# AssemblyAI-Community/MinImagen

Hardware: NVIDIA H100
Metric: denoising steps/sec (SR256 U-Net, batch 32 per GPU per step) (higher is better)
Workload: dtype f16 tensor-core operands, f32 accumulate / residual stream

## Files before the change

include/minimagen_b200.h:

```cpp
#ifndef MINIMAGEN_B200_H_
#define MINIMAGEN_B200_H_

#include <stdint.h>

#ifdef __cplusplus
extern "C" {
#endif

#define MI_ABI_VERSION 2

int mi_abi_version(void);
const char* mi_last_error(void);
int mi_device_ok(void);
int mi_set_launch_mode(int programmatic_dependent_launch);

int mi_pack_conv_weight_f16(const float* w_oihw, int c_out, int c_in, int kh, int kw, float scale, void* out_f16,
                            void* stream);

int mi_pack_conv_weight_dgrad_f16(const float* w_oihw, int c_out, int c_in, int kh, int kw, void* out_f16, void* stream);

int mi_conv2d_igemm_supported(int H, int W, int c_in, int c_out);
int mi_conv2d_igemm_f16(const void* act_f16, int B, int H, int W, int lda, int c_off, int c_in, const void* act2_f16,
                        int lda2, int c_off2, int c_in1, const void* w_f16, int c_out, int kh, int kw, int mode,
                        const float* bias, const float* residual, float* out_f32, void* out_f16, double* out_stats,
                        long long out_sb, long long out_sh, long long out_sw, long long out_sc, int n_valid,
                        int block_n, int* err_flag, void* workspace, long long workspace_bytes, void* stream);
int mi_conv3x3_res1x1_supported(int H, int W, int c_in, int c_out, int x_cin);
int mi_conv3x3_res1x1_f16(const void* act_f16, int B, int H, int W, int lda, int c_in, const void* act2_f16, int lda2,
                          int c_in1, const void* x_f16, int ldx, int x_cin, const void* x2_f16, int ldx2, int x_cin1,
                          const void* w_f16, int c_out, const float* bias, const float* residual, float* out_f32,
                          void* out_f16, double* out_stats, int* err_flag, void* stream);
long long mi_conv2d_igemm_workspace_bytes(void);

int mi_conv3x3_gn_supported(int H, int W, int c0, int c1, int c_out, int groups);
int mi_conv3x3_gn_silu_f16(const float* src0, int c0, const float* src1, int c1, float scale1, int B, int H, int W,
                           int groups, const double* stats0, const double* stats1, const float* gamma,
                           const float* beta, const float* scale_shift, int scale_shift_ld, float eps,
                           const void* w_f16, int c_out, const float* bias, const float* residual, float* out_f32,
                           void* out_f16, double* out_stats, int* err_flag, void* stream);

int mi_conv2d_direct_f32(const float* in, int B, int Hin, int Win, int c_in, int ldi, const float* w_oihw, int c_out,
// ... 104 lines not shown
```

minimagen_b200/_native.py:

```python
import ctypes
import os
from ctypes import c_char_p, c_float, c_int, c_longlong, c_void_p

import torch

_HERE = os.path.dirname(os.path.abspath(__file__))
LIB_PATH = os.path.join(_HERE, "lib", "libminimagen_b200.so")

_P, _I, _L, _F = c_void_p, c_int, c_longlong, c_float

SIGNATURES = {
    "mi_abi_version": [],
    "mi_last_error": [],
    "mi_device_ok": [],
    "mi_set_launch_mode": [_I],
    "mi_pack_conv_weight_f16": [_P, _I, _I, _I, _I, _F, _P, _P],
    "mi_pack_conv_weight_dgrad_f16": [_P, _I, _I, _I, _I, _P, _P],
    "mi_conv2d_igemm_supported": [_I, _I, _I, _I],
    "mi_conv2d_igemm_f16": [_P, _I, _I, _I, _I, _I, _I, _P, _I, _I, _I, _P, _I, _I, _I, _I, _P, _P, _P, _P, _P, _L, _L, _L, _L,
                            _I, _I, _P, _P, _L, _P],
    "mi_conv3x3_res1x1_supported": [_I, _I, _I, _I, _I],
    "mi_conv3x3_res1x1_f16": [_P, _I, _I, _I, _I, _I, _P, _I, _I, _P, _I, _I, _P, _I, _I, _P, _I, _P, _P, _P, _P, _P, _P, _P],
    "mi_conv2d_igemm_workspace_bytes": [],
    "mi_conv3x3_gn_supported": [_I, _I, _I, _I, _I, _I],
    "mi_conv3x3_gn_silu_f16": [_P, _I, _P, _I, _F, _I, _I, _I, _I, _P, _P, _P, _P, _P, _I, _F, _P, _I, _P, _P, _P, _P, _P, _P,
                               _P],
    "mi_conv2d_direct_f32": [_P, _I, _I, _I, _I, _I, _P, _I, _I, _I, _I, _I, _P, _P, _P, _I, _I, _L, _L, _L, _L, _P],
    "mi_gn_stats": [_P, _I, _P, _I, _F, _I, _I, _I, _I, _P, _P],
    "mi_gn_apply_silu": [_P, _I, _P, _I, _F, _I, _I, _I, _I, _P, _I, _P, _I, _P, _P, _P, _I, _F, _P, _I, _P],
    "mi_cast_act": [_P, _I, _P, _I, _F, _I, _I, _I, _I, _I, _P, _I, _P],
    "mi_ln_rows": [_P, _L, _I, _P, _P, _F, _I, _P, _P, _P, _P],
    "mi_linear_f32": [_P, _I, _I, _P, _P, _I, _I, _I, _P, _P, _P, _F, _P],
    "mi_sinusoidal_posemb": [_P, _I, _I, _P, _P],
    "mi_text_tokens": [_P, _I, _I, _I, _P, _P, _P, _I, _P, _I, _I, _P, _P],
    "mi_place_rows": [_P, _I, _I, _I, _P, _I, _I, _P],
# ... 109 lines not shown
```

minimagen_b200/csrc/capi.cu:

```cuda
#include "../../include/minimagen_b200.h"

#include <cuda_runtime.h>
#include <stdio.h>
#include <stdlib.h>
#include <string.h>
#include <string>

#include "conv_tc.cuh"
#include "kernels.cuh"

namespace {

thread_local char g_err[256] = "ok";

int fail(int code, const char* what) {
    snprintf(g_err, sizeof(g_err), "%s (code %d)", what, code);
    return code;
}
int check(int rc, const char* fn) {
    if (rc == 0) return 0;
    if (rc == -1) return fail(rc, (std::string(fn) + ": unsupported shape / alignment").c_str());
    if (rc == -2) {
        cudaError_t e = cudaGetLastError();
        return fail(rc, (std::string(fn) + ": kernel launch failed: " + cudaGetErrorString(e)).c_str());
// ... 27 lines not shown

int mi_pack_conv_weight_dgrad_f16(const float* w, int c_out, int c_in, int kh, int kw, void* out, void* stream) {
    return check(mi::pack_conv_weight_dgrad(w, c_out, c_in, kh, kw, (__half*)out, S(stream)), "mi_pack_conv_weight_dgrad_f16");
}
int mi_pack_conv_weight_f16(const float* w, int c_out, int c_in, int kh, int kw, float scale, void* out, void* stream) {
    return check(mi::pack_conv_weight(w, c_out, c_in, kh, kw, scale, (__half*)out, S(stream)), "mi_pack_conv_weight_f16");
}

int mi_conv2d_igemm_supported(int H, int W, int c_in, int c_out) { return mi::conv_tc_supported(H, W, c_in, c_out) ? 1 : 0; }

static int igemm_common(const void* act, int B, int H, int W, int lda, int c_off, int c_in, const void* act2, int lda2,
                        int c_off2, int c_in1, const void* w, int c_out, int kh, int kw, int mode, const float* bias,
                        const float* residual, float* out_f32, void* out_f16, double* out_stats, long long out_sb,
                        long long out_sh, long long out_sw, long long out_sc, int n_valid, int block_n, int* err_flag,
                        void* workspace, long long workspace_bytes, const void* x_act, int ldx, int x_off, int x_cin,
                        const void* x_act2, int ldx2, int x_off2, int x_cin1, void* stream) {
    mi::ConvTcProblem p{};
    p.x_act = x_act; p.x_lda = ldx; p.x_chan_off = x_off; p.Cx = x_cin;
    p.x_act2 = x_act2; p.x_lda2 = ldx2; p.x_chan_off2 = x_off2; p.Cx1 = x_cin1;
    if (x_act && !(mode == 0 && kh == 3 && kw == 3)) return fail(-9, "mi_conv3x3_res1x1_f16: the folded 1x1 operand needs a 3x3 stride-1 conv");
    (void)workspace; (void)workspace_bytes;
    p.act = act; p.B = B; p.H = H; p.W = W; p.lda = lda; p.a_channels = lda; p.a_chan_off = c_off; p.Cin = c_in;
    p.wpacked = w; p.Cout = c_out;
    p.act2 = act2; p.lda2 = lda2; p.a_chan_off2 = c_off2; p.Cin1 = c_in1; p.stats = out_stats;
    if (out_stats && (out_sc > 1 || (c_out % 32) != 0)) return fail(-8, "mi_conv2d_igemm_f16: out_stats needs channel-contiguous output and c_out % 32 == 0");
    if (out_stats && ((long long)H * W) % 32 != 0)
        return fail(-8, "mi_conv2d_igemm_f16: out_stats needs H*W % 32 == 0 (a warp's output rows must belong to one image)");
    p.out_f32 = out_f32; p.out_f16 = (__half*)out_f16; p.bias = bias; p.residual = residual;
    p.out_sb = out_sb; p.out_sh = out_sh; p.out_sw = out_sw; p.out_sc = out_sc; p.n_valid = n_valid;
    p.block_n_hint = block_n; p.err_flag = err_flag;
    if (mode == 0) {
        if (!(kh & 1) || !(kw & 1) || kh * kw > mi::kConvMaxTaps) return fail(-4, "mi_conv2d_igemm_f16: mode 0 needs odd kh,kw with kh*kw <= 16");
// ... 36 lines not shown
    if (out_sc <= 1 && ((out_sw % 4) || (out_sh % 4) || (out_sb % 4)))
        return fail(-8, "mi_conv2d_igemm_f16: channel-contiguous output strides must be multiples of 4 elements");
    if (out_sc > 1 && residual) return fail(-8, "mi_conv2d_igemm_f16: residual needs channel-contiguous output");
    const int rc = mi::conv_tc_launch(p, S(stream));
    if (rc != 0) return fail(rc, mi::conv_tc_strerror(rc));
    return 0;
}

int mi_conv2d_igemm_f16(const void* act, int B, int H, int W, int lda, int c_off, int c_in, const void* act2, int lda2,
                        int c_off2, int c_in1, const void* w, int c_out, int kh, int kw, int mode, const float* bias,
                        const float* residual, float* out_f32, void* out_f16, double* out_stats, long long out_sb,
                        long long out_sh, long long out_sw, long long out_sc, int n_valid, int block_n, int* err_flag,
                        void* workspace, long long workspace_bytes, void* stream) {
    return igemm_common(act, B, H, W, lda, c_off, c_in, act2, lda2, c_off2, c_in1, w, c_out, kh, kw, mode, bias, residual,
                        out_f32, out_f16, out_stats, out_sb, out_sh, out_sw, out_sc, n_valid, block_n, err_flag, workspace,
                        workspace_bytes, nullptr, 0, 0, 0, nullptr, 0, 0, 0, stream);
}

int mi_conv3x3_res1x1_supported(int H, int W, int c_in, int c_out, int x_cin) {
    const bool t16 = W == 16 && H % 16 == 0, t32 = !t16 && H % 32 == 0 && W % 8 == 0;
    return (t16 || t32) && mi::conv_tc_supported(H, W, c_in, c_out) && x_cin > 0 && x_cin % 64 == 0 && c_out % 128 == 0;
}

int mi_conv3x3_res1x1_f16(const void* act, int B, int H, int W, int lda, int c_in, const void* act2, int lda2, int c_in1,
                          const void* x_act, int ldx, int x_cin, const void* x_act2, int ldx2, int x_cin1, const void* w,
                          int c_out, const float* bias, const float* residual, float* out_f32, void* out_f16,
                          double* out_stats, int* err_flag, void* stream) {
    if (!mi_conv3x3_res1x1_supported(H, W, c_in, c_out, x_cin))
        return fail(-9, "mi_conv3x3_res1x1_f16: unsupported geometry (see mi_conv3x3_res1x1_supported)");
    return igemm_common(act, B, H, W, lda, 0, c_in, act2, lda2, 0, c_in1, w, c_out, 3, 3, 0, bias, residual, out_f32, out_f16,
                        out_stats, (long long)H * W * c_out, (long long)W * c_out, c_out, 1, 0, 0, err_flag, nullptr, 0, x_act,
                        ldx, 0, x_cin, x_act2, ldx2, 0, x_cin1, stream);
}

long long mi_conv2d_igemm_workspace_bytes(void) { return 0; }

int mi_conv3x3_gn_supported(int H, int W, int c0, int c1, int c_out, int groups) {
    return mi::conv_gn_supported(H, W, c0, c1, c_out, groups) ? 1 : 0;
}

int mi_conv3x3_gn_silu_f16(const float* src0, int c0, const float* src1, int c1, float scale1, int B, int H, int W,
                           int groups, const double* stats0, const double* stats1, const float* gamma,
                           const float* beta, const float* scale_shift, int scale_shift_ld, float eps, const void* w,
                           int c_out, const float* bias, const float* residual, float* out_f32, void* out_f16,
                           double* out_stats, int* err_flag, void* stream) {
    mi::ConvGnProblem p{};
    p.src0 = src0; p.C0 = c0; p.src1 = src1; p.C1 = c1; p.scale1 = scale1; p.B = B; p.H = H; p.W = W; p.groups = groups;
// ... 214 lines not shown
```

minimagen_b200/csrc/conv_tc.cu:

```cuda
#include "conv_tc.cuh"

#include <cuda_runtime.h>
#include <mutex>
#include <stdio.h>

#include "kernels.cuh"
#include "launch.cuh"
#include "ptx.cuh"
#include "sat_half.cuh"
#include "wgmma.cuh"

namespace mi {

namespace {

constexpr int kNumThreads = 384;
constexpr uint32_t kABytes = kConvBlockM * kConvBlockK * 2;
constexpr uint32_t kRingBudget = 192 * 1024;
constexpr uint32_t kAuxBytes = 512;
constexpr uint32_t kSmemMax = 227 * 1024;
constexpr int kProducerRegs = 40;
constexpr int kConsumerRegs = 232;
static_assert(128 * kProducerRegs + 256 * kConsumerRegs <= 65536, "register file overcommitted");
constexpr int kTurnBar = 2;
constexpr int kStatBar = 4;
constexpr uint32_t stat_scratch_bytes(int block_n) { return 2 * 4 * (block_n / 16 > 0 ? block_n / 16 : 1) * 2 * 8; }

template <int BLOCK_N>
struct Cfg {
    static constexpr uint32_t kBBytes = BLOCK_N * kConvBlockK * 2;
    static constexpr uint32_t kStageBytes = kABytes + kBBytes;
    static constexpr int kStages = (kRingBudget / kStageBytes) > 8 ? 8 : (kRingBudget / kStageBytes);
    static constexpr uint32_t kSmemBytes = kStages * kStageBytes + 1024  + kAuxBytes;
};

__device__ __forceinline__ float silu(float v) { return __fdividef(v, 1.0f + __expf(-v)); }

template <int BLOCK_N, bool GN>
__global__ void __launch_bounds__(kNumThreads, 1)
conv_wg_kernel(const __grid_constant__ CUtensorMap tmA, const __grid_constant__ CUtensorMap tmA2,
               const __grid_constant__ CUtensorMap tmB, const __grid_constant__ CUtensorMap tmX,
               const __grid_constant__ CUtensorMap tmX2, const __grid_constant__ ConvTcArgs args,
               const __grid_constant__ GnPrologueArgs gn) {
    using C = Cfg<BLOCK_N>;
    constexpr int STAGES = C::kStages;
    static_assert(2 * STAGES * 8 <= 256, "barrier block overlaps the GroupNorm scratch");
    constexpr bool PP = !GN && BLOCK_N <= 128;
    constexpr int HALVES = PP ? 2 : 1;

    extern __shared__ uint8_t smem_raw[];
    uint8_t* smem = reinterpret_cast<uint8_t*>((reinterpret_cast<uintptr_t>(smem_raw) + 1023) & ~uintptr_t(1023));
    uint64_t* bars = reinterpret_cast<uint64_t*>(smem + STAGES * C::kStageBytes);
    uint64_t* full_bar = bars;
    uint64_t* empty_bar = bars + STAGES;

    const int warp = threadIdx.x >> 5;
    const int lane = threadIdx.x & 31;
    const int wg = threadIdx.x >> 7;
    int* err = args.err_flag;

    if (threadIdx.x == 0) {
        ptx::prefetch_tensormap(&tmB);
        if (!GN) {
// ... 22 lines not shown
            if (warp == 0) {
                int stage = 0;
                uint32_t phase = 0;
                for (int tile = blockIdx.x; tile < total_tiles; tile += gridDim.x) {
                    const int nt = tile % args.tiles_n;
                    const int mt = tile / args.tiles_n;
                    const int w0 = (mt % args.tiles_w) * BW;
                    const int h0 = ((mt / args.tiles_w) % args.tiles_h) * BH;
                    const int b0 = (mt / (args.tiles_w * args.tiles_h)) * BB;
                    const int n0 = nt * BLOCK_N;
                    for (int kb = 0; kb < num_kb; ++kb) {
                        ptx::mbar_wait(&empty_bar[stage], phase ^ 1, err, 100 + stage);
                        if (ptx::elect_one()) {
                            uint8_t* sa = smem + stage * C::kStageBytes;
                            uint8_t* sb = sa + kABytes;
                            ptx::mbar_arrive_expect_tx(&full_bar[stage], C::kStageBytes);
                            if (kb < num_tap_kb) {
                                const int t = kb / args.chunks_per_tap, j = kb - t * args.chunks_per_tap;
                                const int cw = w0 * args.in_stride + args.dw[t], ch = h0 * args.in_stride + args.dh[t];
                                if (j < args.a_split)
                                    ptx::tma_load_5d(&tmA, &full_bar[stage], sa, args.a_chan_off + j * kConvBlockK, cw, ch,
                                                     args.ph[t], b0);
                                else
                                    ptx::tma_load_5d(&tmA2, &full_bar[stage], sa,
                                                     args.a_chan_off2 + (j - args.a_split) * kConvBlockK, cw, ch, args.ph[t], b0);
                            } else {
                                const int jx = kb - num_tap_kb;
                                if (jx < args.x_split)
                                    ptx::tma_load_5d(&tmX, &full_bar[stage], sa, args.x_chan_off + jx * kConvBlockK, w0, h0, 0, b0);
                                else
                                    ptx::tma_load_5d(&tmX2, &full_bar[stage], sa,
                                                     args.x_chan_off2 + (jx - args.x_split) * kConvBlockK, w0, h0, 0, b0);
                            }
                            ptx::tma_load_2d(&tmB, &full_bar[stage], sb, kb * kConvBlockK, n0);
                        }
                        if (++stage == STAGES) { stage = 0; phase ^= 1; }
                    }
                }
                pdl_trigger();
            }
        } else {
            float* s_mean = reinterpret_cast<float*>(reinterpret_cast<uint8_t*>(bars) + 256);
            float* s_rstd = s_mean + 32;
            float* sA = reinterpret_cast<float*>(reinterpret_cast<uint8_t*>(bars) + kAuxBytes);
            const int tt = threadIdx.x;
            const int lq = tt & 7;
            const int prow = tt >> 3;
            const int C0 = gn.C0, C1 = gn.C1, Ctot = C0 + C1, Cg = Ctot / gn.groups;
            const int H = args.H, W = args.W;
// ... 120 lines not shown
        if (PP) skip(cw * num_kb);
        int bw_r[2 * HALVES], bh_r[2 * HALVES], bb_r[2 * HALVES], bb_warp[HALVES];
#pragma unroll
        for (int h = 0; h < HALVES; ++h) {
            const int m_warp = (PP ? h : cw) * 64 + wq * 16;
            bb_warp[h] = m_warp >> (args.bw_log2 + args.bh_log2);
#pragma unroll
            for (int r = 0; r < 2; ++r) {
                const int m = m_warp + (lane >> 2) + 8 * r;
                bw_r[2 * h + r] = m & (BW - 1);
                bh_r[2 * h + r] = (m >> args.bw_log2) & (BH - 1);
                bb_r[2 * h + r] = m >> (args.bw_log2 + args.bh_log2);
            }
        }
        constexpr int NQ = BLOCK_N / 16 > 0 ? BLOCK_N / 16 : 1;
        const bool tile_stats = PP && args.stats != nullptr && BB == 1;
        double* st_red = reinterpret_cast<double*>(reinterpret_cast<uint8_t*>(bars) + kAuxBytes);
        const bool vec = args.out_sc == 1 && ((reinterpret_cast<uintptr_t>(args.out_f32) & 7) == 0) &&
                         ((reinterpret_cast<uintptr_t>(args.residual) & 7) == 0) &&
                         ((reinterpret_cast<uintptr_t>(args.out_f16) & 3) == 0);

        for (int tile = blockIdx.x + (PP ? cw : 0) * gridDim.x; tile < total_tiles; tile += (PP ? 2 : 1) * gridDim.x) {
            const int nt = tile % args.tiles_n;
            const int mt = tile / args.tiles_n;
            const int n0 = nt * BLOCK_N;
            if (PP && tile != (int)blockIdx.x) ptx::bar_sync(kTurnBar + cw, 256);
            int prev = -1;
            for (int kb = 0; kb < num_kb; ++kb) {
                ptx::mbar_wait(&full_bar[stage], phase, err, 300 + stage);
                const uint32_t sa = ptx::smem_u32(smem + stage * C::kStageBytes);
                const uint64_t db = ptx::make_sw128_desc(sa + kABytes);
                ptx::wg_fence();
#pragma unroll
                for (int k = 0; k < kConvBlockK / 16; ++k)
#pragma unroll
                    for (int h = 0; h < HALVES; ++h) {
                        const uint64_t da = ptx::make_sw128_desc(sa + (PP ? h : cw) * (64 * 128));
                        ptx::Wgmma<BLOCK_N, 0>::run(acc[h], da + 2 * k, db + 2 * k, (kb | k) != 0);
                    }
                ptx::wg_commit();
                ptx::wg_wait<1>();
                if (prev >= 0 && (threadIdx.x & 127) == 0) ptx::mbar_arrive(&empty_bar[prev]);
                prev = stage;
                if (++stage == STAGES) { stage = 0; phase ^= 1; }
            }
            if (PP && tile + (int)gridDim.x < total_tiles) ptx::bar_arrive(kTurnBar + (cw ^ 1), 256);
            if (PP) skip(num_kb);
            ptx::wg_wait<0>();
#pragma unroll
            for (int h = 0; h < HALVES; ++h) ptx::wg_fence_regs(acc[h]);
            if (prev >= 0 && (threadIdx.x & 127) == 0) ptx::mbar_arrive(&empty_bar[prev]);

            const int tw0 = (mt % args.tiles_w) * BW;
            const int th0 = ((mt / args.tiles_w) % args.tiles_h) * BH;
            const int tb0 = (mt / (args.tiles_w * args.tiles_h)) * BB;
// ... 2 lines not shown
            for (int hf = 0; hf < HALVES; ++hf) {
                bool valid[2];
                long long pix[2];
#pragma unroll
                for (int r = 0; r < 2; ++r) {
                    const int w = tw0 + bw_r[2 * hf + r], h = th0 + bh_r[2 * hf + r], b = tb0 + bb_r[2 * hf + r];
                    valid[r] = (b < args.B) && (h < args.H) && (w < args.W);
                    pix[r] = (long long)b * args.out_sb + (long long)h * args.out_sh + (long long)w * args.out_sw;
                }
                const float* a = acc[hf];
                float st_s[BLOCK_N / 16 > 0 ? BLOCK_N / 16 : 1], st_q[BLOCK_N / 16 > 0 ? BLOCK_N / 16 : 1];
#pragma unroll
                for (int q = 0; q < BLOCK_N / 16; ++q) { st_s[q] = 0.f; st_q[q] = 0.f; }
#pragma unroll
                for (int j = 0; j < BLOCK_N / 8; ++j) {
                    const int n = n0 + 8 * j + cq;
                    if (fast) {
                        float2 bv = make_float2(0.f, 0.f);
                        if (args.bias) bv = __ldg(reinterpret_cast<const float2*>(args.bias + n));
#pragma unroll
                        for (int r = 0; r < 2; ++r) {
                            if (!valid[r]) continue;
                            const long long o = pix[r] + n;
                            float2 f = make_float2(a[4 * j + 2 * r] + bv.x, a[4 * j + 2 * r + 1] + bv.y);
                            if (args.residual) {
                                const float2 rv = *reinterpret_cast<const float2*>(args.residual + o);
                                f.x += rv.x; f.y += rv.y;
                            }
                            st_s[j >> 1] += f.x + f.y;
                            st_q[j >> 1] += f.x * f.x + f.y * f.y;
                            if (args.out_f32) *reinterpret_cast<float2*>(args.out_f32 + o) = f;
// ... 19 lines not shown
                if (args.stats) {
                    const int b_img = tb0 + bb_warp[hf];
                    const bool any = __any_sync(0xffffffffu, valid[0] || valid[1]);
#pragma unroll
                    for (int q = 0; q < BLOCK_N / 16; ++q) {
#pragma unroll
                        for (int o = 1; o <= 16; o <<= 1) {
                            st_s[q] += __shfl_xor_sync(0xffffffffu, st_s[q], o);
                            st_q[q] += __shfl_xor_sync(0xffffffffu, st_q[q], o);
                        }
                        if (lane == 0 && tile_stats) {
                            double* r = st_red + ((cw * 4 + wq) * NQ + q) * 2;
                            r[0] = (hf == 0 ? 0.0 : r[0]) + (double)st_s[q];
                            r[1] = (hf == 0 ? 0.0 : r[1]) + (double)st_q[q];
                        } else if (lane == 0 && any) {
                            double* dst = args.stats + ((long long)b_img * args.stats_blocks + (n0 >> 4) + q) * 2;
                            atomicAdd(dst, (double)st_s[q]);
                            atomicAdd(dst + 1, (double)st_q[q]);
                        }
                    }
                }
            }
            if (tile_stats) {
                ptx::bar_sync(kStatBar + cw, 128);
                if (wq == 0 && lane < NQ) {
                    const double* r = st_red + (cw * 4 * NQ + lane) * 2;
                    double s = r[0], sq = r[1];
#pragma unroll
                    for (int w = 1; w < 4; ++w) { s += r[w * NQ * 2]; sq += r[w * NQ * 2 + 1]; }
                    double* dst = args.stats + ((long long)tb0 * args.stats_blocks + (n0 >> 4) + lane) * 2;
                    atomicAdd(dst, s);
                    atomicAdd(dst + 1, sq);
                }
                ptx::bar_sync(kStatBar + cw, 128);
            }
        }
    }
}


typedef CUresult (*PFN_encodeTiled)(CUtensorMap*, CUtensorMapDataType, cuuint32_t, void*, const cuuint64_t*,
                                    const cuuint64_t*, const cuuint32_t*, const cuuint32_t*, CUtensorMapInterleave,
                                    CUtensorMapSwizzle, CUtensorMapL2promotion, CUtensorMapFloatOOBfill);

PFN_encodeTiled get_encode() {
// ... 66 lines not shown
    return enc(m, CU_TENSOR_MAP_DATA_TYPE_FLOAT16, 5, const_cast<void*>(ptr), gdim, gstr, box, estr,
               CU_TENSOR_MAP_INTERLEAVE_NONE, CU_TENSOR_MAP_SWIZZLE_128B, CU_TENSOR_MAP_L2_PROMOTION_L2_256B,
               CU_TENSOR_MAP_FLOAT_OOB_FILL_NONE);
}

CUresult encode_weights(PFN_encodeTiled enc, CUtensorMap* m, const void* ptr, cuuint64_t K, int Cout, int block_n) {
    cuuint64_t gdim[2] = {K, (cuuint64_t)Cout};
    cuuint64_t gstr[1] = {K * 2};
    cuuint32_t box[2] = {kConvBlockK, (cuuint32_t)block_n};
    cuuint32_t estr[2] = {1, 1};
    return enc(m, CU_TENSOR_MAP_DATA_TYPE_FLOAT16, 2, const_cast<void*>(ptr), gdim, gstr, box, estr,
               CU_TENSOR_MAP_INTERLEAVE_NONE, CU_TENSOR_MAP_SWIZZLE_128B, CU_TENSOR_MAP_L2_PROMOTION_L2_256B,
               CU_TENSOR_MAP_FLOAT_OOB_FILL_NONE);
}

template <int BLOCK_N, bool GN>
int launch(const CUtensorMap& tmA, const CUtensorMap& tmA2, const CUtensorMap& tmB, const CUtensorMap& tmX,
           const CUtensorMap& tmX2, const ConvTcArgs& args, const GnPrologueArgs& gn, uint32_t extra_smem,
           cudaStream_t stream) {
    using C = Cfg<BLOCK_N>;
    static bool attr_set = false;
    if (!attr_set) {
        if (cudaFuncSetAttribute(conv_wg_kernel<BLOCK_N, GN>, cudaFuncAttributeMaxDynamicSharedMemorySize, kSmemMax) !=
            cudaSuccess)
            return -10;
        attr_set = true;
    }
    const int total_tiles = args.tiles_w * args.tiles_h * args.tiles_b * args.tiles_n;
    const int num_sms = num_sms_of_current_device();
    const int grid = total_tiles < num_sms ? total_tiles : num_sms;
    const uint32_t smem = C::kSmemBytes + (!GN && BLOCK_N <= 128 ? stat_scratch_bytes(BLOCK_N) : 0u) + extra_smem;
    launch_k(conv_wg_kernel<BLOCK_N, GN>, grid, kNumThreads, smem, stream, tmA, tmA2, tmB, tmX, tmX2, args, gn);
    return cudaGetLastError() == cudaSuccess ? 0 : -11;
}

}

PFN_tmaEncodeTiled get_tma_encode() { return get_encode(); }

const char* conv_tc_strerror(int code) {
    switch (code) {
        case 0: return "ok";
        case -1: return "conv_tc: C_in (per tap) must be a positive multiple of 64";
        case -2: return "conv_tc: C_out must be a multiple of 16";
        case -3: return "conv_tc: W must be a power of two >= 8 or a multiple of 128; H*W tiling unsupported";
        case -4: return "conv_tc: too many taps (max 16)";
        case -5: return "conv_tc: cuTensorMapEncodeTiled unavailable";
        case -6: return "conv_tc: tensor map encode failed (activations)";
        case -7: return "conv_tc: tensor map encode failed (weights)";
        case -8: return "conv_tc: pointer/stride alignment (16 B) violated";
        case -9: return "conv_tc: the folded 1x1 operand needs a stride-1 conv over one phase";
        case -10: return "conv_tc: cudaFuncSetAttribute(max dynamic smem) failed";
        case -11: return "conv_tc: kernel launch failed";
        default: return "conv_tc: unknown error";
    }
}

bool conv_tc_supported(int H, int W, int Cin, int Cout) {
    if (Cin <= 0 || Cin % kConvBlockK != 0 || Cout <= 0 || Cout % 16 != 0) return false;
    if (W >= 128) return true;
    if (ilog2_exact(W) < 3) return false;
    const int bh = 128 / W;
    if (H >= bh) return H % bh == 0;
    return ilog2_exact(H) >= 0;
}

int conv_tc_launch(const ConvTcProblem& p, cudaStream_t stream) {
    if (p.Cin <= 0 || p.Cin % kConvBlockK != 0) return -1;
// ... 9 lines not shown
    ConvTcArgs a{};
    a.num_taps = p.num_taps;
    a.chunks_per_tap = p.Cin / kConvBlockK;
    tile_geometry(p.H, p.W, p.B, a);
    a.a_chan_off = p.a_chan_off;
    a.in_stride = p.in_stride == 2 ? 2 : 1;
    a.out_sb = p.out_sb; a.out_sh = p.out_sh; a.out_sw = p.out_sw;
    a.out_sc = p.out_sc > 0 ? p.out_sc : 1;
    a.n_valid = p.n_valid > 0 ? p.n_valid : p.Cout;
    a.out_f32 = p.out_f32; a.out_f16 = p.out_f16; a.bias = p.bias; a.residual = p.residual;
    a.err_flag = p.err_flag;
    a.stats = p.stats; a.stats_blocks = p.Cout / 16;
    for (int t = 0; t < p.num_taps; ++t) { a.dh[t] = p.dh[t]; a.dw[t] = p.dw[t]; a.ph[t] = p.ph[t]; }

    const int tiles_m = a.tiles_w * a.tiles_h * a.tiles_b;
    const int block_n = pick_block_n(p.Cout, tiles_m, p.block_n_hint, num_sms_of_current_device());
    a.tiles_n = p.Cout / block_n;

    CUtensorMap tmA, tmA2, tmB, tmX, tmX2;
    a.a_split = (p.act2 ? p.Cin1 : p.Cin) / kConvBlockK;
    a.a_chan_off2 = p.a_chan_off2;
    if (encode_act(enc, &tmA, p.act, p.a_channels, p.lda, p.W, p.H, p.phases, p.B, a.in_stride, a) != CUDA_SUCCESS) return -6;
    tmA2 = tmA;
    if (p.act2) {
        if (p.Cin1 <= 0 || p.Cin1 % kConvBlockK || p.Cin1 >= p.Cin || (p.lda2 % 8) || (reinterpret_cast<uintptr_t>(p.act2) & 15) ||
            a.in_stride != 1)
            return -8;
        if (encode_act(enc, &tmA2, p.act2, p.lda2, p.lda2, p.W, p.H, p.phases, p.B, 1, a) != CUDA_SUCCESS) return -6;
    }
    tmX = tmA; tmX2 = tmA;
    if (p.x_act) {
// ... 1 lines not shown
        if (p.Cx <= 0 || p.Cx % kConvBlockK || (p.x_lda % 8) || (reinterpret_cast<uintptr_t>(p.x_act) & 15)) return -8;
        if (p.x_act2 && (p.Cx1 <= 0 || p.Cx1 % kConvBlockK || p.Cx1 >= p.Cx || (p.x_lda2 % 8) ||
                         (reinterpret_cast<uintptr_t>(p.x_act2) & 15)))
            return -8;
        a.x_chunks = p.Cx / kConvBlockK;
        a.x_split = (p.x_act2 ? p.Cx1 : p.Cx) / kConvBlockK;
        a.x_chan_off = p.x_chan_off; a.x_chan_off2 = p.x_chan_off2;
        if (encode_act(enc, &tmX, p.x_act, p.x_lda, p.x_lda, p.W, p.H, 1, p.B, 1, a) != CUDA_SUCCESS) return -6;
        tmX2 = tmX;
        if (p.x_act2 && encode_act(enc, &tmX2, p.x_act2, p.x_lda2, p.x_lda2, p.W, p.H, 1, p.B, 1, a) != CUDA_SUCCESS) return -6;
    }
    const cuuint64_t K = (cuuint64_t)p.num_taps * p.Cin + (p.x_act ? (cuuint64_t)p.Cx : 0);
    if (encode_weights(enc, &tmB, p.wpacked, K, p.Cout, block_n) != CUDA_SUCCESS) return -7;

    const GnPrologueArgs gn{};
    switch (block_n) {
        case 256: return launch<256, false>(tmA, tmA2, tmB, tmX, tmX2, a, gn, 0, stream);
        case 128: return launch<128, false>(tmA, tmA2, tmB, tmX, tmX2, a, gn, 0, stream);
        case 64: return launch<64, false>(tmA, tmA2, tmB, tmX, tmX2, a, gn, 0, stream);
        case 32: return launch<32, false>(tmA, tmA2, tmB, tmX, tmX2, a, gn, 0, stream);
        default: return launch<16, false>(tmA, tmA2, tmB, tmX, tmX2, a, gn, 0, stream);
    }
}


bool conv_gn_supported(int H, int W, int C0, int C1, int Cout, int groups) {
    const int C = C0 + C1;
    if (H <= 0 || W <= 0 || H % 32 || W % 8 || C0 <= 0 || C0 % 64 || C1 < 0 || C1 % 64 || Cout <= 0 || Cout % 128) return false;
    if (!conv_tc_supported(H, W, C, Cout) || H * W < kConvBlockM) return false;
    if (groups < 1 || groups > 32 || C % groups) return false;
// ... 41 lines not shown
```

minimagen_b200/csrc/conv_tc.cuh:

```cuda
#pragma once
#include <cuda_fp16.h>
#include <cuda_runtime.h>
#include <stdint.h>

namespace mi {

constexpr int kConvBlockM = 128;
constexpr int kConvBlockK = 64;
constexpr int kConvMaxTaps = 16;

struct ConvTcArgs {
    int num_taps, chunks_per_tap;
    int bw_log2, bh_log2;
    int tiles_w, tiles_h, tiles_b, tiles_n;
    int B, H, W;
    int a_chan_off;
    int in_stride;
    int a_split, a_chan_off2;
    int x_chunks, x_split;
    int x_chan_off, x_chan_off2;
    long long out_sb, out_sh, out_sw;
    long long out_sc;
    int n_valid;
    float* out_f32;
    __half* out_f16;
    const float* bias;
    const float* residual;
    int* err_flag;
    double* stats;
    int stats_blocks;
    int8_t dh[kConvMaxTaps], dw[kConvMaxTaps], ph[kConvMaxTaps];
};

struct ConvTcProblem {
    const void* act;
    int B, H, W;
    int phases;
    int in_stride;
    int lda;
    int a_channels;
    int a_chan_off;
    int Cin;
    const void* act2;
    int lda2, a_chan_off2, Cin1;
    const void* wpacked;
    int Cout;
    const void* x_act; int x_lda, x_chan_off, Cx;
    const void* x_act2; int x_lda2, x_chan_off2, Cx1;
    int num_taps;
    int8_t dh[kConvMaxTaps], dw[kConvMaxTaps], ph[kConvMaxTaps];
    float* out_f32; __half* out_f16; const float* bias; const float* residual;
    long long out_sb, out_sh, out_sw;
    long long out_sc;
    int n_valid;
    int block_n_hint;
    double* stats;
    int* err_flag;
};

struct GnPrologueArgs {
    const float* src0;
    const float* src1;
    int C0, C1, groups;
    float scale1, eps;
    const double* stats0;
    const double* stats1;
    const float* gamma;
    const float* beta;
    const float* scale_shift;
    int ss_ld;
};

// ... 22 lines not shown
```

minimagen_b200/layers.py:

```python
import math
import os

import torch
from torch import nn

from .helpers import default, exists
from .ops import get_ops

F16, F32, F64 = torch.float16, torch.float32, torch.float64


STATS_BLOCK = 16

GN_INPUT_F32 = True

FUSE_GN_CONV = {"0": False, "1": True, "pair": "pair", "all": "all"}.get(os.environ.get("MI_FUSE_GN_CONV", "0"), False)
FUSE_OVER_FOLD = os.environ.get("MI_FUSE_OVER_FOLD", "1") == "1"


def fuse_block_ok(c_out):
    if not FUSE_GN_CONV:
        return False
    if FUSE_GN_CONV == 'all':
        return True
# ... 462 lines not shown

class _UpsampleSeq(nn.Sequential):

    def run(self, x):
        return self[1].run(x, upsample=True, f32=GN_INPUT_F32, f16=True, stats=True)

    def forward(self, x):
        _no_grad_check(x)
        return to_nchw(self.run(to_nhwc(x)).need_f32())


def Upsample(dim, dim_out=None):
    return _UpsampleSeq(nn.Upsample(scale_factor=2, mode='nearest'), Conv2d(dim, default(dim_out, dim), 3, padding=1))


class CrossEmbedLayer(nn.Module):

    def __init__(self, dim_in, kernel_sizes, dim_out=None, stride=2):
        super().__init__()
        assert all((k % 2) == (stride % 2) for k in kernel_sizes)
        dim_out = default(dim_out, dim_in)
        kernel_sizes = sorted(kernel_sizes)
        num_scales = len(kernel_sizes)
        dim_scales = [int(dim_out / (2 ** i)) for i in range(1, num_scales)]
        dim_scales = [*dim_scales, dim_out - sum(dim_scales)]
        self.dim_in, self.dim_out, self.stride = dim_in, dim_out, stride
        self.convs = nn.ModuleList([
            Conv2d(dim_in, ds, k, stride=stride, padding=(k - stride) // 2) for k, ds in zip(kernel_sizes, dim_scales)])

    def stem_tc_ok(self, H, W):
# ... 2 lines not shown
                and get_ops().igemm_supported(H, W, 128, self.dim_out))

    def _stem_weights(self):
        key = tuple((c.weight.data_ptr(), c.weight._version, c.bias._version) for c in self.convs)
        if getattr(self, "_stem_key", None) != key:
            dev = self.convs[0].weight.device
            wm = torch.zeros((self.dim_out, 15, 16, 8), dtype=F32, device=dev)
            off = 0
            for conv in self.convs:
                k, n = conv.kernel_size[0], conv.out_channels
                lo = 7 - k // 2
                wm[off:off + n, lo:lo + k, lo:lo + k, :self.dim_in] = conv.weight.detach().permute(0, 2, 3, 1)
                off += n
            self._stem_w = wm.reshape(self.dim_out, 15 * 128).to(F16).contiguous()
            self._stem_b = torch.cat([c.bias.detach() for c in self.convs]).contiguous()
            self._stem_key = key
        return self._stem_w, self._stem_b

    def run_stem(self, x, lowres=None):
        ops = get_ops()
        B, Cx, H, W = x.shape
        Cl = lowres.shape[1] if exists(lowres) else 0
        assert Cx + Cl == self.dim_in
        x = x.to(F32).contiguous()
        lowres = lowres.to(F32).contiguous() if exists(lowres) else None
        if self.stem_tc_ok(H, W):
            a = torch.empty((B, 1, H, W, 128), dtype=F16, device=x.device)
            ops.stem_unroll(x, Cx, lowres, Cl, B, H, W, a)
            wp, bias = self._stem_weights()
            C = self.dim_out
            out = torch.empty((B, H, W, C), dtype=F32, device=x.device)
            out16 = torch.empty((B, 1, H, W, C), dtype=F16, device=x.device)
            st = stats_zeros((B, C // STATS_BLOCK, 2), x.device) if (C % 32 == 0 and (H * W) % 32 == 0) else None
            ops.conv_igemm(a, B, H, W, 128, 0, 128, wp, C, 15, 1, 0, bias, None, out, out16, (H * W * C, W * C, C),
                           out_stats=st)
            return Act(out, out16, st)
        cp = (self.dim_in + 3) // 4 * 4
        x_pad = torch.empty((B, H, W, cp), dtype=F32, device=x.device)
        ops.nchw_to_nhwc(x, Cx, lowres, Cl, B, H * W, cp, x_pad)
        return Act(f32=self.run_padded(x_pad, B, H, W))

    def run_padded(self, x_pad, B, H, W):
        assert self.stride == 1
        ops = get_ops()
        out = torch.empty((B, H, W, self.dim_out), dtype=F32, device=x_pad.device)
        C = self.dim_out
        off = 0
        for conv in self.convs:
            k = conv.kernel_size[0]
            ops.conv_direct(x_pad, B, H, W, self.dim_in, x_pad.shape[3], conv.weight.detach(), conv.out_channels, k, k,
# ... 285 lines not shown
```

minimagen_b200/ops.py:

```python
import torch

from . import _native as N

F16, F32, F64, I64, U8 = torch.float16, torch.float32, torch.float64, torch.int64, torch.uint8


def _chk(t, dtype, name):
    if t is None:
        return
    if t.dtype != dtype:
        raise TypeError(f"{name}: expected {dtype}, got {t.dtype}")
    if not t.is_contiguous():
        raise ValueError(f"{name}: tensor must be contiguous")


def _chk_out(t, dtype, name):
    if t is not None and t.dtype != dtype:
        raise TypeError(f"{name}: expected {dtype}, got {t.dtype}")


class NativeOps:
    name = "native-sm90a"
    attention_tc = True

    def set_launch_mode(self, pdl):
        N.load().mi_set_launch_mode(int(bool(pdl)))

    def igemm_supported(self, H, W, c_in, c_out):
        return bool(N.load().mi_conv2d_igemm_supported(int(H), int(W), int(c_in), int(c_out)))

    def pack_conv_weight(self, w, scale=1.0):
        if w.dim() == 2:
            w = w[:, :, None, None]
        w = w.detach().to(F32).contiguous()
        O, I, KH, KW = w.shape
        out = torch.empty((O, KH * KW * I), dtype=F16, device=w.device)
        N.call("mi_pack_conv_weight_f16", N.ptr(w), O, I, KH, KW, float(scale), N.ptr(out), N.stream())
        return out

    def pack_conv_weight_dgrad(self, w):
        if w.dim() == 2:
            w = w[:, :, None, None]
        w = w.detach().to(F32).contiguous()
        O, I, KH, KW = w.shape
        out = torch.empty((I, KH * KW * O), dtype=F16, device=w.device)
        N.call("mi_pack_conv_weight_dgrad_f16", N.ptr(w), O, I, KH, KW, N.ptr(out), N.stream())
        return out

    def conv_igemm(self, act, B, H, W, lda, c_off, c_in, wp, c_out, kh, kw, mode, bias, residual, out_f32, out_f16,
                   out_strides, block_n=0, out_sc=1, n_valid=0, act2=None, lda2=0, c_off2=0, c_in1=0, out_stats=None):
        _chk(act, F16, "act"); _chk(act2, F16, "act2"); _chk(wp, F16, "wp"); _chk(bias, F32, "bias")
        _chk_out(residual, F32, "residual"); _chk_out(out_f32, F32, "out_f32"); _chk_out(out_f16, F16, "out_f16")
        _chk(out_stats, F64, "out_stats")
        sb, sh, sw = out_strides
        N.call("mi_conv2d_igemm_f16", N.ptr(act), B, H, W, lda, c_off, c_in, N.ptr(act2), lda2, c_off2, c_in1,
               N.ptr(wp), c_out, kh, kw, mode, N.ptr(bias), N.ptr(residual), N.ptr(out_f32), N.ptr(out_f16),
               N.ptr(out_stats), sb, sh, sw, out_sc, n_valid, block_n, None, None, 0, N.stream())

    def conv_res1x1_supported(self, H, W, c_in, c_out, x_cin):
        return bool(N.load().mi_conv3x3_res1x1_supported(int(H), int(W), int(c_in), int(c_out), int(x_cin)))

    def conv_res1x1(self, act, B, H, W, lda, c_in, act2, lda2, c_in1, x, ldx, x_cin, x2, ldx2, x_cin1, wp, c_out, bias,
                    residual, out_f32, out_f16, out_stats):
        for nm, t in (("act", act), ("act2", act2), ("x", x), ("x2", x2), ("wp", wp)):
            _chk(t, F16, nm)
        _chk(bias, F32, "bias"); _chk(residual, F32, "residual"); _chk(out_f32, F32, "out_f32"); _chk(out_f16, F16, "out_f16")
        _chk(out_stats, F64, "out_stats")
        N.call("mi_conv3x3_res1x1_f16", N.ptr(act), B, H, W, lda, c_in, N.ptr(act2), lda2, c_in1, N.ptr(x), ldx, x_cin,
               N.ptr(x2), ldx2, x_cin1, N.ptr(wp), c_out, N.ptr(bias), N.ptr(residual), N.ptr(out_f32), N.ptr(out_f16),
# ... 289 lines not shown
```

Before: 12.06.

## Skip zero weight column blocks in CrossEmbed stem conv via per-k-block windows

Adds a column-window variant of the implicit-GEMM conv kernel. A host-side table records, for each 64-wide k-block, the first output-channel group with non-zero weights. The kernel then loads only the live quarter or half of the B tile and issues narrower WGMMAs, with swapped column mapping in the epilogue and stats. This targets the CrossEmbed stem, whose concatenated multi-kernel-size weights are structurally zero in many k-blocks, to cut tensor-core and TMA work. It forces a single full-width N tile, which may reduce parallelism, and it adds a template instantiation.

```diff
diff --git a/include/minimagen_b200.h b/include/minimagen_b200.h
--- a/include/minimagen_b200.h
+++ b/include/minimagen_b200.h
@@ -25,6 +25,12 @@
                         const float* bias, const float* residual, float* out_f32, void* out_f16, double* out_stats,
                         long long out_sb, long long out_sh, long long out_sw, long long out_sc, int n_valid,
                         int block_n, int* err_flag, void* workspace, long long workspace_bytes, void* stream);
+int mi_conv2d_igemm_cols_f16(const void* act_f16, int B, int H, int W, int lda, int c_off, int c_in,
+                             const void* act2_f16, int lda2, int c_off2, int c_in1, const void* w_f16, int c_out, int kh,
+                             int kw, int mode, const float* bias, const float* residual, float* out_f32, void* out_f16,
+                             double* out_stats, long long out_sb, long long out_sh, long long out_sw, long long out_sc,
+                             int n_valid, int block_n, const int* kb_live_from_host, int kb_count, int* err_flag,
+                             void* stream);
 int mi_conv3x3_res1x1_supported(int H, int W, int c_in, int c_out, int x_cin);
 int mi_conv3x3_res1x1_f16(const void* act_f16, int B, int H, int W, int lda, int c_in, const void* act2_f16, int lda2,
                           int c_in1, const void* x_f16, int ldx, int x_cin, const void* x2_f16, int ldx2, int x_cin1,
diff --git a/minimagen_b200/_native.py b/minimagen_b200/_native.py
--- a/minimagen_b200/_native.py
+++ b/minimagen_b200/_native.py
@@ -19,6 +19,8 @@
     "mi_conv2d_igemm_supported": [_I, _I, _I, _I],
     "mi_conv2d_igemm_f16": [_P, _I, _I, _I, _I, _I, _I, _P, _I, _I, _I, _P, _I, _I, _I, _I, _P, _P, _P, _P, _P, _L, _L, _L, _L,
                             _I, _I, _P, _P, _L, _P],
+    "mi_conv2d_igemm_cols_f16": [_P, _I, _I, _I, _I, _I, _I, _P, _I, _I, _I, _P, _I, _I, _I, _I, _P, _P, _P, _P, _P, _L, _L,
+                                 _L, _L, _I, _I, _P, _I, _P, _P],
     "mi_conv3x3_res1x1_supported": [_I, _I, _I, _I, _I],
     "mi_conv3x3_res1x1_f16": [_P, _I, _I, _I, _I, _I, _P, _I, _I, _P, _I, _I, _P, _I, _I, _P, _I, _P, _P, _P, _P, _P, _P, _P],
     "mi_conv2d_igemm_workspace_bytes": [],
diff --git a/minimagen_b200/csrc/capi.cu b/minimagen_b200/csrc/capi.cu
--- a/minimagen_b200/csrc/capi.cu
+++ b/minimagen_b200/csrc/capi.cu
@@ -65,8 +65,10 @@
                         const float* residual, float* out_f32, void* out_f16, double* out_stats, long long out_sb,
                         long long out_sh, long long out_sw, long long out_sc, int n_valid, int block_n, int* err_flag,
                         void* workspace, long long workspace_bytes, const void* x_act, int ldx, int x_off, int x_cin,
-                        const void* x_act2, int ldx2, int x_off2, int x_cin1, void* stream) {
+                        const void* x_act2, int ldx2, int x_off2, int x_cin1, const int* kb_live_from, int kb_live_len,
+                        void* stream) {
     mi::ConvTcProblem p{};
+    p.kb_live_from = kb_live_from; p.kb_live_len = kb_live_len;
     p.x_act = x_act; p.x_lda = ldx; p.x_chan_off = x_off; p.Cx = x_cin;
     p.x_act2 = x_act2; p.x_lda2 = ldx2; p.x_chan_off2 = x_off2; p.Cx1 = x_cin1;
     if (x_act && !(mode == 0 && kh == 3 && kw == 3)) return fail(-9, "mi_conv3x3_res1x1_f16: the folded 1x1 operand needs a 3x3 stride-1 conv");
@@ -133,7 +135,18 @@
                         void* workspace, long long workspace_bytes, void* stream) {
     return igemm_common(act, B, H, W, lda, c_off, c_in, act2, lda2, c_off2, c_in1, w, c_out, kh, kw, mode, bias, residual,
                         out_f32, out_f16, out_stats, out_sb, out_sh, out_sw, out_sc, n_valid, block_n, err_flag, workspace,
-                        workspace_bytes, nullptr, 0, 0, 0, nullptr, 0, 0, 0, stream);
+                        workspace_bytes, nullptr, 0, 0, 0, nullptr, 0, 0, 0, nullptr, 0, stream);
+}
+
+int mi_conv2d_igemm_cols_f16(const void* act, int B, int H, int W, int lda, int c_off, int c_in, const void* act2,
+                             int lda2, int c_off2, int c_in1, const void* w, int c_out, int kh, int kw, int mode,
+                             const float* bias, const float* residual, float* out_f32, void* out_f16, double* out_stats,
+                             long long out_sb, long long out_sh, long long out_sw, long long out_sc, int n_valid,
+                             int block_n, const int* kb_live_from, int kb_count, int* err_flag, void* stream) {
+    if (!kb_live_from) return fail(-12, "mi_conv2d_igemm_cols_f16: kb_live_from is required");
+    return igemm_common(act, B, H, W, lda, c_off, c_in, act2, lda2, c_off2, c_in1, w, c_out, kh, kw, mode, bias, residual,
+                        out_f32, out_f16, out_stats, out_sb, out_sh, out_sw, out_sc, n_valid, block_n, err_flag, nullptr, 0,
+                        nullptr, 0, 0, 0, nullptr, 0, 0, 0, kb_live_from, kb_count, stream);
 }
 
 int mi_conv3x3_res1x1_supported(int H, int W, int c_in, int c_out, int x_cin) {
@@ -149,7 +162,7 @@
         return fail(-9, "mi_conv3x3_res1x1_f16: unsupported geometry (see mi_conv3x3_res1x1_supported)");
     return igemm_common(act, B, H, W, lda, 0, c_in, act2, lda2, 0, c_in1, w, c_out, 3, 3, 0, bias, residual, out_f32, out_f16,
                         out_stats, (long long)H * W * c_out, (long long)W * c_out, c_out, 1, 0, 0, err_flag, nullptr, 0, x_act,
-                        ldx, 0, x_cin, x_act2, ldx2, 0, x_cin1, stream);
+                        ldx, 0, x_cin, x_act2, ldx2, 0, x_cin1, nullptr, 0, stream);
 }
 
 long long mi_conv2d_igemm_workspace_bytes(void) { return 0; }
diff --git a/minimagen_b200/csrc/conv_tc.cu b/minimagen_b200/csrc/conv_tc.cu
--- a/minimagen_b200/csrc/conv_tc.cu
+++ b/minimagen_b200/csrc/conv_tc.cu
@@ -3,6 +3,7 @@
 #include <cuda_runtime.h>
 #include <mutex>
 #include <stdio.h>
+#include <type_traits>
 
 #include "kernels.cuh"
 #include "launch.cuh"
@@ -36,7 +37,7 @@
 
 __device__ __forceinline__ float silu(float v) { return __fdividef(v, 1.0f + __expf(-v)); }
 
-template <int BLOCK_N, bool GN>
+template <int BLOCK_N, bool GN, bool WIN = false>
 __global__ void __launch_bounds__(kNumThreads, 1)
 conv_wg_kernel(const __grid_constant__ CUtensorMap tmA, const __grid_constant__ CUtensorMap tmA2,
                const __grid_constant__ CUtensorMap tmB, const __grid_constant__ CUtensorMap tmX,
@@ -47,6 +48,7 @@
     static_assert(2 * STAGES * 8 <= 256, "barrier block overlaps the GroupNorm scratch");
     constexpr bool PP = !GN && BLOCK_N <= 128;
     constexpr int HALVES = PP ? 2 : 1;
+    static_assert(!WIN || (PP && (BLOCK_N == 64 || BLOCK_N == 128)), "column windows need a 64- or 128-wide ping-pong tile");
 
     extern __shared__ uint8_t smem_raw[];
     uint8_t* smem = reinterpret_cast<uint8_t*>((reinterpret_cast<uintptr_t>(smem_raw) + 1023) & ~uintptr_t(1023));
@@ -99,7 +101,9 @@
                         if (ptx::elect_one()) {
                             uint8_t* sa = smem + stage * C::kStageBytes;
                             uint8_t* sb = sa + kABytes;
-                            ptx::mbar_arrive_expect_tx(&full_bar[stage], C::kStageBytes);
+                            int live = 4;
+                            if constexpr (WIN) live = ((args.win_quarter >> kb) & 1) ? 1 : ((args.win_half >> kb) & 1) ? 2 : 4;
+                            ptx::mbar_arrive_expect_tx(&full_bar[stage], kABytes + live * (C::kBBytes / 4));
                             if (kb < num_tap_kb) {
                                 const int t = kb / args.chunks_per_tap, j = kb - t * args.chunks_per_tap;
                                 const int cw = w0 * args.in_stride + args.dw[t], ch = h0 * args.in_stride + args.dh[t];
@@ -117,7 +121,13 @@
                                     ptx::tma_load_5d(&tmX2, &full_bar[stage], sa,
                                                      args.x_chan_off2 + (jx - args.x_split) * kConvBlockK, w0, h0, 0, b0);
                             }
-                            ptx::tma_load_2d(&tmB, &full_bar[stage], sb, kb * kConvBlockK, n0);
+                            if constexpr (WIN) {
+                                for (int g = 4 - live; g < 4; ++g)
+                                    ptx::tma_load_2d(&tmB, &full_bar[stage], sb + (3 - g) * (C::kBBytes / 4), kb * kConvBlockK,
+                                                     n0 + g * (BLOCK_N / 4));
+                            } else {
+                                ptx::tma_load_2d(&tmB, &full_bar[stage], sb, kb * kConvBlockK, n0);
+                            }
                         }
                         if (++stage == STAGES) { stage = 0; phase ^= 1; }
                     }
@@ -268,6 +278,7 @@
             }
         }
         constexpr int NQ = BLOCK_N / 16 > 0 ? BLOCK_N / 16 : 1;
+        constexpr int SWAP = WIN ? 3 * BLOCK_N / 4 : 0;
         const bool tile_stats = PP && args.stats != nullptr && BB == 1;
         double* st_red = reinterpret_cast<double*>(reinterpret_cast<uint8_t*>(bars) + kAuxBytes);
         const bool vec = args.out_sc == 1 && ((reinterpret_cast<uintptr_t>(args.out_f32) & 7) == 0) &&
@@ -279,20 +290,37 @@
             const int mt = tile / args.tiles_n;
             const int n0 = nt * BLOCK_N;
             if (PP && tile != (int)blockIdx.x) ptx::bar_sync(kTurnBar + cw, 256);
+            if constexpr (WIN) {
+#pragma unroll
+                for (int h = 0; h < HALVES; ++h)
+#pragma unroll
+                    for (int i = 0; i < BLOCK_N / 2; ++i) acc[h][i] = 0.f;
+            }
             int prev = -1;
             for (int kb = 0; kb < num_kb; ++kb) {
                 ptx::mbar_wait(&full_bar[stage], phase, err, 300 + stage);
                 const uint32_t sa = ptx::smem_u32(smem + stage * C::kStageBytes);
-                const uint64_t db = ptx::make_sw128_desc(sa + kABytes);
-                ptx::wg_fence();
-#pragma unroll
-                for (int k = 0; k < kConvBlockK / 16; ++k)
-#pragma unroll
-                    for (int h = 0; h < HALVES; ++h) {
-                        const uint64_t da = ptx::make_sw128_desc(sa + (PP ? h : cw) * (64 * 128));
-                        ptx::Wgmma<BLOCK_N, 0>::run(acc[h], da + 2 * k, db + 2 * k, (kb | k) != 0);
-                    }
-                ptx::wg_commit();
+                auto mma_kb = [&](auto live) {
+                    constexpr int NW = decltype(live)::value;
+                    const uint64_t db = ptx::make_sw128_desc(sa + kABytes);
+                    ptx::wg_fence();
+#pragma unroll
+                    for (int k = 0; k < kConvBlockK / 16; ++k)
+#pragma unroll
+                        for (int h = 0; h < HALVES; ++h) {
+                            const uint64_t da = ptx::make_sw128_desc(sa + (PP ? h : cw) * (64 * 128));
+                            float(&d)[NW / 2] = *reinterpret_cast<float(*)[NW / 2]>(&acc[h][0]);
+                            ptx::Wgmma<NW, 0>::run(d, da + 2 * k, db + 2 * k, (kb | k) != 0);
+                        }
+                    ptx::wg_commit();
+                };
+                if constexpr (WIN) {
+                    if ((args.win_quarter >> kb) & 1) mma_kb(std::integral_constant<int, BLOCK_N / 4>{});
+                    else if ((args.win_half >> kb) & 1) mma_kb(std::integral_constant<int, BLOCK_N / 2>{});
+                    else mma_kb(std::integral_constant<int, BLOCK_N>{});
+                } else {
+                    mma_kb(std::integral_constant<int, BLOCK_N>{});
+                }
                 ptx::wg_wait<1>();
                 if (prev >= 0 && (threadIdx.x & 127) == 0) ptx::mbar_arrive(&empty_bar[prev]);
                 prev = stage;
@@ -325,7 +353,7 @@
                 for (int q = 0; q < BLOCK_N / 16; ++q) { st_s[q] = 0.f; st_q[q] = 0.f; }
 #pragma unroll
                 for (int j = 0; j < BLOCK_N / 8; ++j) {
-                    const int n = n0 + 8 * j + cq;
+                    const int n = n0 + ((8 * j + cq) ^ SWAP);
                     if (fast) {
                         float2 bv = make_float2(0.f, 0.f);
                         if (args.bias) bv = __ldg(reinterpret_cast<const float2*>(args.bias + n));
@@ -375,7 +403,7 @@
                             r[0] = (hf == 0 ? 0.0 : r[0]) + (double)st_s[q];
                             r[1] = (hf == 0 ? 0.0 : r[1]) + (double)st_q[q];
                         } else if (lane == 0 && any) {
-                            double* dst = args.stats + ((long long)b_img * args.stats_blocks + (n0 >> 4) + q) * 2;
+                            double* dst = args.stats + ((long long)b_img * args.stats_blocks + (n0 >> 4) + (q ^ (SWAP >> 4))) * 2;
                             atomicAdd(dst, (double)st_s[q]);
                             atomicAdd(dst + 1, (double)st_q[q]);
                         }
@@ -389,7 +417,7 @@
                     double s = r[0], sq = r[1];
 #pragma unroll
                     for (int w = 1; w < 4; ++w) { s += r[w * NQ * 2]; sq += r[w * NQ * 2 + 1]; }
-                    double* dst = args.stats + ((long long)tb0 * args.stats_blocks + (n0 >> 4) + lane) * 2;
+                    double* dst = args.stats + ((long long)tb0 * args.stats_blocks + (n0 >> 4) + (lane ^ (SWAP >> 4))) * 2;
                     atomicAdd(dst, s);
                     atomicAdd(dst + 1, sq);
                 }
@@ -486,15 +514,15 @@
                CU_TENSOR_MAP_FLOAT_OOB_FILL_NONE);
 }
 
-template <int BLOCK_N, bool GN>
+template <int BLOCK_N, bool GN, bool WIN = false>
 int launch(const CUtensorMap& tmA, const CUtensorMap& tmA2, const CUtensorMap& tmB, const CUtensorMap& tmX,
            const CUtensorMap& tmX2, const ConvTcArgs& args, const GnPrologueArgs& gn, uint32_t extra_smem,
            cudaStream_t stream) {
     using C = Cfg<BLOCK_N>;
     static bool attr_set = false;
     if (!attr_set) {
-        if (cudaFuncSetAttribute(conv_wg_kernel<BLOCK_N, GN>, cudaFuncAttributeMaxDynamicSharedMemorySize, kSmemMax) !=
-            cudaSuccess)
+        if (cudaFuncSetAttribute(conv_wg_kernel<BLOCK_N, GN, WIN>, cudaFuncAttributeMaxDynamicSharedMemorySize,
+                                 kSmemMax) != cudaSuccess)
             return -10;
         attr_set = true;
     }
@@ -502,8 +530,13 @@
     const int num_sms = num_sms_of_current_device();
     const int grid = total_tiles < num_sms ? total_tiles : num_sms;
     const uint32_t smem = C::kSmemBytes + (!GN && BLOCK_N <= 128 ? stat_scratch_bytes(BLOCK_N) : 0u) + extra_smem;
-    launch_k(conv_wg_kernel<BLOCK_N, GN>, grid, kNumThreads, smem, stream, tmA, tmA2, tmB, tmX, tmX2, args, gn);
+    launch_k(conv_wg_kernel<BLOCK_N, GN, WIN>, grid, kNumThreads, smem, stream, tmA, tmA2, tmB, tmX, tmX2, args, gn);
     return cudaGetLastError() == cudaSuccess ? 0 : -11;
+}
+
+int window_code(int live_from, int block_n) {
+    const int live = block_n - (live_from < 0 ? 0 : live_from > block_n ? block_n : live_from);
+    return live <= block_n / 4 ? 2 : live <= block_n / 2 ? 1 : 0;
 }
 
 }
@@ -524,6 +557,8 @@
         case -9: return "conv_tc: the folded 1x1 operand needs a stride-1 conv over one phase";
         case -10: return "conv_tc: cudaFuncSetAttribute(max dynamic smem) failed";
         case -11: return "conv_tc: kernel launch failed";
+        case -12: return "conv_tc: the column-window table must have one entry per k-block, at most 64";
+        case -13: return "conv_tc: column windows need one 64- or 128-wide tile across C_out";
         default: return "conv_tc: unknown error";
     }
 }
@@ -563,7 +598,9 @@
     for (int t = 0; t < p.num_taps; ++t) { a.dh[t] = p.dh[t]; a.dw[t] = p.dw[t]; a.ph[t] = p.ph[t]; }
 
     const int tiles_m = a.tiles_w * a.tiles_h * a.tiles_b;
-    const int block_n = pick_block_n(p.Cout, tiles_m, p.block_n_hint, num_sms_of_current_device());
+    int block_n = pick_block_n(p.Cout, tiles_m, p.block_n_hint, num_sms_of_current_device());
+    if (p.kb_live_from && (p.block_n_hint == 0 || p.block_n_hint == p.Cout || p.block_n_hint == -p.Cout))
+        block_n = p.Cout;
     a.tiles_n = p.Cout / block_n;
 
     CUtensorMap tmA, tmA2, tmB, tmX, tmX2;
@@ -595,6 +632,19 @@
     if (encode_weights(enc, &tmB, p.wpacked, K, p.Cout, block_n) != CUDA_SUCCESS) return -7;
 
     const GnPrologueArgs gn{};
+    if (p.kb_live_from) {
+        const int num_kb = (int)(K / kConvBlockK);
+        if (p.kb_live_len != num_kb || num_kb > kConvMaxWindowKb) return -12;
+        if (block_n != p.Cout || (block_n != 64 && block_n != 128)) return -13;
+        if (encode_weights(enc, &tmB, p.wpacked, K, p.Cout, block_n / 4) != CUDA_SUCCESS) return -7;
+        for (int kb = 0; kb < num_kb; ++kb) {
+            const int q = window_code(p.kb_live_from[kb], block_n);
+            if (q == 1) a.win_half |= 1ull << kb;
+            if (q == 2) a.win_quarter |= 1ull << kb;
+        }
+        if (block_n == 128) return launch<128, false, true>(tmA, tmA2, tmB, tmX, tmX2, a, gn, 0, stream);
+        return launch<64, false, true>(tmA, tmA2, tmB, tmX, tmX2, a, gn, 0, stream);
+    }
     switch (block_n) {
         case 256: return launch<256, false>(tmA, tmA2, tmB, tmX, tmX2, a, gn, 0, stream);
         case 128: return launch<128, false>(tmA, tmA2, tmB, tmX, tmX2, a, gn, 0, stream);
diff --git a/minimagen_b200/csrc/conv_tc.cuh b/minimagen_b200/csrc/conv_tc.cuh
--- a/minimagen_b200/csrc/conv_tc.cuh
+++ b/minimagen_b200/csrc/conv_tc.cuh
@@ -8,6 +8,7 @@
 constexpr int kConvBlockM = 128;
 constexpr int kConvBlockK = 64;
 constexpr int kConvMaxTaps = 16;
+constexpr int kConvMaxWindowKb = 64;
 
 struct ConvTcArgs {
     int num_taps, chunks_per_tap;
@@ -30,6 +31,7 @@
     double* stats;
     int stats_blocks;
     int8_t dh[kConvMaxTaps], dw[kConvMaxTaps], ph[kConvMaxTaps];
+    unsigned long long win_half, win_quarter;
 };
 
 struct ConvTcProblem {
@@ -56,6 +58,8 @@
     int block_n_hint;
     double* stats;
     int* err_flag;
+    const int* kb_live_from;
+    int kb_live_len;
 };
 
 struct GnPrologueArgs {
diff --git a/minimagen_b200/layers.py b/minimagen_b200/layers.py
--- a/minimagen_b200/layers.py
+++ b/minimagen_b200/layers.py
@@ -500,6 +500,15 @@
     return _UpsampleSeq(nn.Upsample(scale_factor=2, mode='nearest'), Conv2d(dim, default(dim_out, dim), 3, padding=1))
 
 
+def kb_live_from(wp, group=32):
+    c_out, K = wp.shape
+    if K % 64 or c_out % group:
+        raise ValueError(f"kb_live_from: need K % 64 == 0 and C_out % {group} == 0, got {tuple(wp.shape)}")
+    live = wp.reshape(c_out // group, group, K // 64, 64).ne(0).any(dim=3).any(dim=1).cpu()
+    first = torch.where(live.any(dim=0), live.int().argmax(dim=0), torch.full((K // 64,), c_out // group))
+    return (first * group).to(torch.int32).contiguous()
+
+
 class CrossEmbedLayer(nn.Module):
 
     def __init__(self, dim_in, kernel_sizes, dim_out=None, stride=2):
@@ -532,6 +541,7 @@
                 off += n
             self._stem_w = wm.reshape(self.dim_out, 15 * 128).to(F16).contiguous()
             self._stem_b = torch.cat([c.bias.detach() for c in self.convs]).contiguous()
+            self._stem_live = kb_live_from(self._stem_w) if self.dim_out % 32 == 0 else None
             self._stem_key = key
         return self._stem_w, self._stem_b
 
@@ -550,8 +560,12 @@
             out = torch.empty((B, H, W, C), dtype=F32, device=x.device)
             out16 = torch.empty((B, 1, H, W, C), dtype=F16, device=x.device)
             st = stats_zeros((B, C // STATS_BLOCK, 2), x.device) if (C % 32 == 0 and (H * W) % 32 == 0) else None
-            ops.conv_igemm(a, B, H, W, 128, 0, 128, wp, C, 15, 1, 0, bias, None, out, out16, (H * W * C, W * C, C),
-                           out_stats=st)
+            strides = (H * W * C, W * C, C)
+            if getattr(ops, "column_windows", False) and self._stem_live is not None and C in (64, 128):
+                ops.conv_igemm(a, B, H, W, 128, 0, 128, wp, C, 15, 1, 0, bias, None, out, out16, strides, out_stats=st,
+                               kb_live_from=self._stem_live)
+            else:
+                ops.conv_igemm(a, B, H, W, 128, 0, 128, wp, C, 15, 1, 0, bias, None, out, out16, strides, out_stats=st)
             return Act(out, out16, st)
         cp = (self.dim_in + 3) // 4 * 4
         x_pad = torch.empty((B, H, W, cp), dtype=F32, device=x.device)
diff --git a/minimagen_b200/ops.py b/minimagen_b200/ops.py
--- a/minimagen_b200/ops.py
+++ b/minimagen_b200/ops.py
@@ -22,6 +22,7 @@
 class NativeOps:
     name = "native-sm90a"
     attention_tc = True
+    column_windows = True
 
     def set_launch_mode(self, pdl):
         N.load().mi_set_launch_mode(int(bool(pdl)))
@@ -48,11 +49,20 @@
         return out
 
     def conv_igemm(self, act, B, H, W, lda, c_off, c_in, wp, c_out, kh, kw, mode, bias, residual, out_f32, out_f16,
-                   out_strides, block_n=0, out_sc=1, n_valid=0, act2=None, lda2=0, c_off2=0, c_in1=0, out_stats=None):
+                   out_strides, block_n=0, out_sc=1, n_valid=0, act2=None, lda2=0, c_off2=0, c_in1=0, out_stats=None,
+                   kb_live_from=None):
         _chk(act, F16, "act"); _chk(act2, F16, "act2"); _chk(wp, F16, "wp"); _chk(bias, F32, "bias")
         _chk_out(residual, F32, "residual"); _chk_out(out_f32, F32, "out_f32"); _chk_out(out_f16, F16, "out_f16")
         _chk(out_stats, F64, "out_stats")
         sb, sh, sw = out_strides
+        if kb_live_from is not None:
+            if kb_live_from.dtype != torch.int32 or kb_live_from.device.type != "cpu" or not kb_live_from.is_contiguous():
+                raise TypeError("kb_live_from: expected a contiguous CPU int32 tensor")
+            N.call("mi_conv2d_igemm_cols_f16", N.ptr(act), B, H, W, lda, c_off, c_in, N.ptr(act2), lda2, c_off2, c_in1,
+                   N.ptr(wp), c_out, kh, kw, mode, N.ptr(bias), N.ptr(residual), N.ptr(out_f32), N.ptr(out_f16),
+                   N.ptr(out_stats), sb, sh, sw, out_sc, n_valid, block_n, kb_live_from.data_ptr(), kb_live_from.numel(),
+                   None, N.stream())
+            return
         N.call("mi_conv2d_igemm_f16", N.ptr(act), B, H, W, lda, c_off, c_in, N.ptr(act2), lda2, c_off2, c_in1,
                N.ptr(wp), c_out, kh, kw, mode, N.ptr(bias), N.ptr(residual), N.ptr(out_f32), N.ptr(out_f16),
                N.ptr(out_stats), sb, sh, sw, out_sc, n_valid, block_n, None, None, 0, N.stream())
```

New measurement: 12.09 (median of 6 runs). No clear change (+0.3%).
